# alibaba/TePDist

Hardware: AMD Instinct MI355X
Metric: tokens/sec (higher is better)
Workload: dtype bf16; 1 GPU; model=gpt2-345m, global_batch=64, seq_len=1024, parallelism=auto-planned-graph:dp1tp1pp1mesh[]micro1

## Files before the change

tepdist_amd/ops/csrc/bindings.cpp:

```cpp

#include <pybind11/pybind11.h>

#include <hip/hip_runtime.h>

#include "common.h"
#include "gemm_plan.h"
#include "kernels.h"

namespace py = pybind11;
using namespace tepdist;

namespace {

hipStream_t S(uintptr_t s) { return reinterpret_cast<hipStream_t>(s); }

void check_launch() { HIP_CHECK(hipGetLastError()); }

}

PYBIND11_MODULE(_tepdist_hip, m) {
  m.doc() = "TePDist-AMD gfx950 kernel library";

  m.def("gemm", [](uintptr_t A, uintptr_t B, uintptr_t C, uintptr_t Cpre,
                   uintptr_t bias, int M, int N, int K, int lda, int ldb,
                   int ldc, int64_t sa, int64_t sb, int64_t sc, int batch,
                   bool a_kc, bool b_kc, int epi, uintptr_t splitk_ws,
                   uintptr_t stream) {
    gemm_bf16(reinterpret_cast<void*>(A), reinterpret_cast<void*>(B),
              reinterpret_cast<void*>(C), reinterpret_cast<void*>(Cpre),
              reinterpret_cast<void*>(bias), M, N, K, lda, ldb, ldc, sa, sb,
              sc, batch, a_kc, b_kc, epi, reinterpret_cast<float*>(splitk_ws),
              S(stream));
    check_launch();
  });

  m.def("gemm_plan", [](int M, int N, int K, int lda, int ldb, bool a_kc,
                        bool b_kc, int epi, int batch) {
    const GemmPlan p = gemm_plan(M, N, K, lda, ldb, a_kc, b_kc, epi, batch);
    return py::make_tuple(p.kernel, p.split_k, p.k_chunk,
                          p.why_not ? p.why_not : "");
  }, py::arg("M"), py::arg("N"), py::arg("K"), py::arg("lda"),
     py::arg("ldb"), py::arg("a_kc") = true, py::arg("b_kc") = true,
     py::arg("epi") = 0, py::arg("batch") = 1);

  m.def("transpose", [](uintptr_t in, uintptr_t out, int R, int C,
                        int64_t si, int64_t so, int batch,
                        uintptr_t stream) {
    transpose_bf16(reinterpret_cast<void*>(in), reinterpret_cast<void*>(out),
                   R, C, si, so, batch, S(stream));
    check_launch();
  });

  m.def("layernorm_fwd", [](uintptr_t x, uintptr_t g, uintptr_t b, uintptr_t y,
                            uintptr_t mean, uintptr_t rstd, int rows, int cols,
                            float eps, uintptr_t stream, uintptr_t res,
                            uintptr_t sum_out) {
    layernorm_fwd_bf16(reinterpret_cast<void*>(x), reinterpret_cast<void*>(g),
                       reinterpret_cast<void*>(b), reinterpret_cast<void*>(y),
                       reinterpret_cast<float*>(mean),
                       reinterpret_cast<float*>(rstd), rows, cols, eps,
                       S(stream), reinterpret_cast<void*>(res),
                       reinterpret_cast<void*>(sum_out));
    check_launch();
  }, pybind11::arg("x"), pybind11::arg("g"), pybind11::arg("b"),
     pybind11::arg("y"), pybind11::arg("mean"), pybind11::arg("rstd"),
     pybind11::arg("rows"), pybind11::arg("cols"), pybind11::arg("eps"),
     pybind11::arg("stream"), pybind11::arg("res") = 0,
     pybind11::arg("sum_out") = 0);

  m.def("layernorm_bwd", [](uintptr_t dy, uintptr_t x, uintptr_t g,
                            uintptr_t mean, uintptr_t rstd, uintptr_t dx,
                            uintptr_t dg_part, uintptr_t db_part,
                            uintptr_t dgamma, uintptr_t dbeta, int rows,
                            int cols, int part_rows, uintptr_t stream,
                            uintptr_t dsum) {
    layernorm_bwd_bf16(reinterpret_cast<void*>(dy), reinterpret_cast<void*>(x),
                       reinterpret_cast<void*>(g),
                       reinterpret_cast<float*>(mean),
                       reinterpret_cast<float*>(rstd),
                       reinterpret_cast<void*>(dx),
                       reinterpret_cast<float*>(dg_part),
                       reinterpret_cast<float*>(db_part), rows, cols,
                       part_rows, S(stream), reinterpret_cast<void*>(dsum));
    check_launch();
    layernorm_bwd_reduce(reinterpret_cast<float*>(dg_part),
                         reinterpret_cast<float*>(db_part),
                         reinterpret_cast<void*>(dgamma),
// ... 299 lines not shown
```

tepdist_amd/ops/csrc/gemm.hip:

```cpp

#include <algorithm>
#include <stdexcept>
#include <string>

#include "common.h"
#include "gemm_tile.h"
#include "kernels.h"

namespace tepdist {

namespace {

constexpr int BM = plan::T128, BN = plan::T128, BK = plan::BK;
constexpr int SLOT = BM * BK;
constexpr int NTHREADS = 256;

DEV_INLINE int lds_off(int row, int col_e) { return loff<BK>(row, col_e); }


DEV_INLINE void stage_kc_load(const bf16_t* __restrict__ src, int F, int K,
                              int ld, int f0, int k0, bool aligned,
                              bf16x8 regs[4]) {
#pragma unroll
  for (int u = 0; u < 4; ++u) {
// ... 188 lines not shown
#pragma unroll
      for (int i = 0; i < 4; ++i) {
        af[i] = frag(sa, wm + i * 16, lane, kk);
        bfr[i] = frag(sb, wn + i * 16, lane, kk);
      }
#pragma unroll
      for (int mi = 0; mi < 4; ++mi)
#pragma unroll
        for (int ni = 0; ni < 4; ++ni)
          acc[mi][ni] = __builtin_amdgcn_mfma_f32_16x16x32_bf16(
              af[mi], bfr[ni], acc[mi][ni], 0, 0, 0);
    }

    if (t + 1 < nk) write_tiles(cur ^ 1, kbeg + (t + 1) * BK);
    __syncthreads();
  }

  float bv[4];
  if (EPI == EPI_BIAS || EPI == EPI_BIAS_GELU) {
#pragma unroll
    for (int ni = 0; ni < 4; ++ni) {
      const int n = n0 + wn + ni * 16 + (lane & 15);
      bv[ni] = (n < N) ? bf2f(bias[n]) : 0.0f;
    }
  }
#pragma unroll
  for (int mi = 0; mi < 4; ++mi) {
#pragma unroll
    for (int ni = 0; ni < 4; ++ni) {
      const int n = n0 + wn + ni * 16 + (lane & 15);
      if (n >= N) continue;
#pragma unroll
      for (int e = 0; e < 4; ++e) {
        const int m = m0 + wm + mi * 16 + (lane >> 4) * 4 + e;
        if (m >= M) continue;
        float v = acc[mi][ni][e];
        if (EPI == EPI_BIAS || EPI == EPI_BIAS_GELU) v += bv[ni];
        const int64_t off = (int64_t)m * ldc + n;
        if (F32OUT) {
          Cf[off] = v;
          continue;
        }
        if (EPI >= 2) {
          const bf16_t pre = f2bf(v);
          Cpre[off] = pre;
          v = gelu_f(bf2f(pre));
        }
        C[off] = f2bf(v);
      }
    }
  }
}

__global__ void splitk_reduce_kernel(const float* __restrict__ parts,
                                     bf16_t* __restrict__ out, int nparts,
                                     int64_t mn) {
  const int64_t stride = (int64_t)gridDim.x * blockDim.x * 4;
  for (int64_t i = ((int64_t)blockIdx.x * blockDim.x + threadIdx.x) * 4;
       i < mn; i += stride) {
    if (i + 4 <= mn) {
      f32x4 sv = *reinterpret_cast<const f32x4*>(parts + i);
      for (int p = 1; p < nparts; ++p) {
        const f32x4 v = *reinterpret_cast<const f32x4*>(parts + p * mn + i);
#pragma unroll
        for (int e = 0; e < 4; ++e) sv[e] += v[e];
      }
      bf16x4 o;
#pragma unroll
      for (int e = 0; e < 4; ++e) o[e] = f2bf(sv[e]);
      *reinterpret_cast<bf16x4*>(out + i) = o;
    } else {
      for (int64_t j = i; j < mn; ++j) {
        float acc = 0.f;
        for (int p = 0; p < nparts; ++p) acc += parts[p * mn + j];
        out[j] = f2bf(acc);
      }
    }
  }
}

void splitk_reduce(const float* parts, bf16_t* out, int nparts, int64_t mn,
                   hipStream_t stream) {
  const int blocks = (int)std::min<int64_t>(
      (mn / 4 + NTHREADS - 1) / NTHREADS, 2048);
  hipLaunchKernelGGL(splitk_reduce_kernel, dim3(std::max(blocks, 1)),
                     dim3(NTHREADS), 0, stream, parts, out, nparts, mn);
}

}

void gemm_bf16(const void* A, const void* B, void* C, void* c_pre,
               const void* bias, int M, int N, int K, int lda, int ldb,
               int ldc, int64_t stride_a, int64_t stride_b, int64_t stride_c,
               int batch, bool a_kc, bool b_kc, int epi, float* splitk_ws,
               hipStream_t stream) {
  const GemmPlan p = gemm_plan(M, N, K, lda, ldb, a_kc, b_kc, epi, batch);
  if (p.kernel == 0)
    throw std::runtime_error(std::string("gemm_bf16: ") + p.why_not);

  const bool split = p.split_k > 1;
  const int64_t mn = (int64_t)M * N;
  if (split && splitk_ws == nullptr)
    throw std::runtime_error("gemm_bf16: split-K plan needs a workspace of " +
                             std::to_string(p.split_k * mn) + " floats");
  if (split && ldc != N)
    throw std::runtime_error("gemm_bf16: split-K plan needs ldc == N");
  void* out = C;
  if (split) {
    out = splitk_ws;
    stride_c = mn;
  }

  if (p.kernel == plan::T256) {
    gemm256_bf16(A, B, out, c_pre, bias, M, N, K, lda, ldb, ldc, stride_a,
                 stride_b, stride_c, batch, !a_kc, epi, p.split_k,
                 p.k_chunk, stream);
  } else {
    const int nbx = (N + BN - 1) / BN, nby = (M + BM - 1) / BM;
    const dim3 grid(nbx * nby, 1, split ? p.split_k : batch), block(NTHREADS);
    const bf16_t* a = static_cast<const bf16_t*>(A);
    const bf16_t* b = static_cast<const bf16_t*>(B);
    bf16_t* cp = static_cast<bf16_t*>(c_pre);
    const bf16_t* bi = static_cast<const bf16_t*>(bias);
#define GEMM_LAUNCH(AKC, BKC, E, F32)                                       \
    hipLaunchKernelGGL((gemm_kernel<AKC, BKC, E, F32>), grid, block, 0,     \
                       stream, a, b, out, cp, bi, M, N, K, lda, ldb, ldc,   \
                       stride_a, stride_b, stride_c, p.k_chunk)
#define GEMM_EPI(AKC, BKC)                                                  \
    if (split) { GEMM_LAUNCH(AKC, BKC, 0, true); }                          \
    else switch (epi) {                  \
      case EPI_NONE: GEMM_LAUNCH(AKC, BKC, EPI_NONE, false); break;         \
      case EPI_BIAS: GEMM_LAUNCH(AKC, BKC, EPI_BIAS, false); break;         \
      case EPI_BIAS_GELU: GEMM_LAUNCH(AKC, BKC, EPI_BIAS_GELU, false); break; \
      case EPI_GELU: GEMM_LAUNCH(AKC, BKC, EPI_GELU, false); break;         \
    }
    if (a_kc && b_kc) { GEMM_EPI(true, true); }
    else if (a_kc && !b_kc) { GEMM_EPI(true, false); }
    else if (!a_kc && b_kc) { GEMM_EPI(false, true); }
    else { GEMM_EPI(false, false); }
#undef GEMM_EPI
#undef GEMM_LAUNCH
  }
  if (split) {
    HIP_CHECK(hipGetLastError());
    splitk_reduce(splitk_ws, static_cast<bf16_t*>(C), p.split_k, mn, stream);
  }
}

}
```

tepdist_amd/ops/csrc/gemm256.hip:

```cpp

#include <stdexcept>

#include "common.h"
#include "gemm_tile.h"
#include "kernels.h"

namespace tepdist {

namespace {

constexpr int BM = plan::T256, BN = plan::T256, BK = plan::BK;
constexpr int NTH = 512;
constexpr int QROWS = 64;
constexpr int SLOT_E = QROWS * BK;

DEV_INLINE int qoff(int row, int col_e) { return loff<BK>(row, col_e); }

DEV_INLINE void stage_q(const bf16_t* __restrict__ src, int64_t ld, int f0,
                        int k0, bf16_t* dst) {
  const int wave = threadIdx.x >> 6;
  const int row = threadIdx.x >> 3;
  const int c = (threadIdx.x & 7) * 8;
  const int ksrc = k0 + (c ^ (SWZ8(row) << 3));
  const bf16_t* g = src + (int64_t)(f0 + row) * ld + ksrc;
// ... 4 lines not shown
DEV_INLINE int qoff_f32(int row, int col_e) {
  return row * BK + (col_e ^ (SWZ8(row) << 2));
}

DEV_INLINE bf16x8 fragq(const bf16_t* slot, int row, int col_e) {
  return *reinterpret_cast<const bf16x8*>(slot + qoff(row, col_e));
}

typedef unsigned int u32x2 __attribute__((ext_vector_type(2)));
typedef __attribute__((address_space(3))) const bf16_t* lds_cptr_t;

template <int OFF>
DEV_INLINE bf16x4 tr_read_asm(uint32_t addr) {
  u32x2 v;
  asm volatile("ds_read_b64_tr_b16 %0, %1 offset:%2"
               : "=v"(v)
               : "v"(addr), "n"(OFF)
               : "memory");
  return __builtin_bit_cast(bf16x4, v);
}

template <int KK>
DEV_INLINE bf16x8 tr_frag_asm(const bf16_t* slot, int df, int lane) {
  const int i = lane & 15, g = lane >> 4;
  const uint32_t addr = (uint32_t)(uintptr_t)(lds_cptr_t)(
      slot + qoff(4 * g + (i >> 2), 16 * df + 4 * (i & 3)));
  const bf16x4 lo = tr_read_asm<KK * 32 * BK * 2>(addr);
  const bf16x4 hi = tr_read_asm<(KK * 32 + 16) * BK * 2>(addr);
  bf16x8 f;
#pragma unroll
  for (int e = 0; e < 4; ++e) {
    f[e] = lo[e];
    f[e + 4] = hi[e];
  }
  return f;
}

template <bool KO, int KK>
DEV_INLINE bf16x8 frag_fk(const bf16_t* slot, int df, int lane) {
  if (KO) return tr_frag_asm<KK>(slot, df, lane);
  return fragq(slot, df * 16 + (lane & 15), 8 * (lane >> 4) + 32 * KK);
}

#define RAW_BAR() __builtin_amdgcn_s_barrier()
#define VMCNT6() asm volatile("s_waitcnt vmcnt(6)" ::: "memory")
#define LGKM_WAIT_KO()                                      \
  do {                                                      \
    if (KO) {                                               \
      asm volatile("s_waitcnt lgkmcnt(0)" ::: "memory");    \
      __builtin_amdgcn_sched_barrier(0);                    \
    }                                                       \
  } while (0)

template <int EPI, bool F32OUT = false, bool KO = false>
__launch_bounds__(NTH, 1) __global__
void gemm256_kernel(const bf16_t* __restrict__ A,
                    const bf16_t* __restrict__ B, void* __restrict__ Cv,
                    bf16_t* __restrict__ Cpre,
                    const bf16_t* __restrict__ bias, int M, int N, int K,
                    int lda, int ldb, int ldc, int64_t strideA,
                    int64_t strideB, int64_t strideC, int k_chunk) {
  bf16_t* C = static_cast<bf16_t*>(Cv);
  float* Cf = static_cast<float*>(Cv);
  int kbeg = 0, kend = K;
  if (F32OUT) {
    kbeg = blockIdx.z * k_chunk;
    kend = min(K, kbeg + k_chunk);
    Cf += blockIdx.z * strideC;
    if (kend <= kbeg) kbeg = kend = 0;
  } else {
    A += blockIdx.z * strideA;
    B += blockIdx.z * strideB;
    C += blockIdx.z * strideC;
    if (EPI >= 2) Cpre += blockIdx.z * strideC;
  }

  const int nbx = N / BN;
  const int swz = xcd_remap(blockIdx.x, gridDim.x);
  const int m0 = (swz / nbx) * BM, n0 = (swz % nbx) * BN;

  __shared__ bf16_t smem[16 * SLOT_E];
  bf16_t* const aslot = smem;
  bf16_t* const bslot = smem + 8 * SLOT_E;

  const int lane = threadIdx.x & 63;
  const int wm = (threadIdx.x >> 8) & 1;
  const int wn = (threadIdx.x >> 6) & 3;

  f32x4 acc[8][4] = {};

  const int nk = (kend - kbeg) / BK;

  auto stage_1 = [&](const bf16_t* __restrict__ src, int ld, int f0, int t,
                     bf16_t* dst) {
    if (KO) stage_q(src, ld, kbeg + t * BK, f0, dst);
    else    stage_q(src, ld, f0, kbeg + t * BK, dst);
  };
  auto stage_a = [&](int t, int q2) {
    stage_1(A, lda, m0 + 64 * q2, t, aslot + ((4 * t + q2) & 7) * SLOT_E);
    stage_1(A, lda, m0 + 64 * (q2 + 1), t,
            aslot + ((4 * t + q2 + 1) & 7) * SLOT_E);
  };
  auto stage_b = [&](int t, int q2) {
    stage_1(B, ldb, n0 + 64 * q2, t, bslot + ((4 * t + q2) & 7) * SLOT_E);
    stage_1(B, ldb, n0 + 64 * (q2 + 1), t,
            bslot + ((4 * t + q2 + 1) & 7) * SLOT_E);
  };

  if (nk > 0) {
    stage_a(0, 0);
    stage_a(0, 2);
    stage_b(0, 0);
    stage_b(0, 2);
    if (nk > 1) {
      stage_a(1, 0);
      stage_a(1, 2);
      stage_b(1, 0);
    }
    VMCNT6();
  }
  RAW_BAR();

  bf16x8 af[8][2];
  for (int t = 0; t < nk; ++t) {
    if (t + 1 == nk && nk > 1) {
      asm volatile("s_waitcnt vmcnt(0)" ::: "memory");
      RAW_BAR();
    }
    {
      const bf16_t* as0 = aslot + ((4 * t + 2 * wm) & 7) * SLOT_E;
      const bf16_t* as1 = aslot + ((4 * t + 2 * wm + 1) & 7) * SLOT_E;
#pragma unroll
      for (int mi = 0; mi < 8; ++mi) {
        const bf16_t* s = (mi < 4) ? as0 : as1;
        af[mi][0] = frag_fk<KO, 0>(s, mi & 3, lane);
        af[mi][1] = frag_fk<KO, 1>(s, mi & 3, lane);
      }
      bf16x8 bf0[2];
      {
        const bf16_t* bs = bslot + ((4 * t + 0) & 7) * SLOT_E;
        bf0[0] = frag_fk<KO, 0>(bs, wn, lane);
        bf0[1] = frag_fk<KO, 1>(bs, wn, lane);
      }
      if (t + 1 < nk) stage_b(t + 1, 2);
      RAW_BAR();
      LGKM_WAIT_KO();
      __builtin_amdgcn_s_setprio(1);
#pragma unroll
      for (int mi = 0; mi < 8; ++mi)
#pragma unroll
        for (int kk = 0; kk < 2; ++kk)
          acc[mi][0] = __builtin_amdgcn_mfma_f32_16x16x32_bf16(
              af[mi][kk], bf0[kk], acc[mi][0], 0, 0, 0);
      __builtin_amdgcn_s_setprio(0);
      RAW_BAR();
    }
#pragma unroll
    for (int p = 1; p < 4; ++p) {
      bf16x8 bfp[2];
      {
        const bf16_t* bs = bslot + ((4 * t + p) & 7) * SLOT_E;
        bfp[0] = frag_fk<KO, 0>(bs, wn, lane);
        bfp[1] = frag_fk<KO, 1>(bs, wn, lane);
      }
      if (p == 1 && t + 2 < nk) stage_a(t + 2, 0);
      if (p == 2 && t + 2 < nk) stage_a(t + 2, 2);
      if (p == 3 && t + 2 < nk) stage_b(t + 2, 0);
      RAW_BAR();
      LGKM_WAIT_KO();
      __builtin_amdgcn_s_setprio(1);
#pragma unroll
      for (int mi = 0; mi < 8; ++mi)
#pragma unroll
        for (int kk = 0; kk < 2; ++kk)
          acc[mi][p] = __builtin_amdgcn_mfma_f32_16x16x32_bf16(
              af[mi][kk], bfp[kk], acc[mi][p], 0, 0, 0);
      __builtin_amdgcn_s_setprio(0);
      if (p == 3) VMCNT6();
      RAW_BAR();
    }
  }

  float bv[4];
  if (EPI == EPI_BIAS || EPI == EPI_BIAS_GELU) {
#pragma unroll
    for (int p = 0; p < 4; ++p)
      bv[p] = bf2f(bias[n0 + 64 * p + wn * 16 + (lane & 15)]);
  }
  if (!F32OUT) {
    asm volatile("s_waitcnt lgkmcnt(0)" ::: "memory");
    __builtin_amdgcn_s_barrier();
    bf16_t* img = smem;
#pragma unroll
    for (int p = 0; p < 4; ++p) {
      const int cl = wn * 16 + (lane & 15);
#pragma unroll
      for (int mi = 0; mi < 8; ++mi)
#pragma unroll
        for (int e = 0; e < 4; ++e) {
          const int row = wm * 128 + mi * 16 + (lane >> 4) * 4 + e;
          float v = acc[mi][p][e];
          if (EPI == EPI_BIAS || EPI == EPI_BIAS_GELU) v += bv[p];
          img[qoff(row, cl)] = f2bf(v);
        }
      asm volatile("s_waitcnt lgkmcnt(0)" ::: "memory");
      __builtin_amdgcn_s_barrier();
      const int sr = threadIdx.x >> 3;
      const int c8 = (threadIdx.x & 7) * 8;
#pragma unroll
      for (int rr = 0; rr < BM; rr += 64) {
        const int row = rr + sr;
        const int64_t off = (int64_t)(m0 + row) * ldc + n0 + 64 * p + c8;
        bf16x8 v8 = *reinterpret_cast<const bf16x8*>(img + qoff(row, c8));
        if (EPI == EPI_DGELU) {
          const bf16x8 pv = *reinterpret_cast<const bf16x8*>(Cpre + off);
#pragma unroll
          for (int e = 0; e < 8; ++e)
            v8[e] = f2bf(bf2f(v8[e]) * gelu_grad_f(bf2f(pv[e])));
        } else if (EPI >= 2) {
          *reinterpret_cast<bf16x8*>(Cpre + off) = v8;
#pragma unroll
          for (int e = 0; e < 8; ++e) v8[e] = f2bf(gelu_f(bf2f(v8[e])));
        }
        *reinterpret_cast<bf16x8*>(C + off) = v8;
      }
      asm volatile("s_waitcnt lgkmcnt(0)" ::: "memory");
      __builtin_amdgcn_s_barrier();
    }
    return;
  }
  asm volatile("s_waitcnt lgkmcnt(0)" ::: "memory");
  __builtin_amdgcn_s_barrier();
  {
    float* imgf = reinterpret_cast<float*>(smem);
#pragma unroll
    for (int p = 0; p < 4; ++p) {
      const int cl = wn * 16 + (lane & 15);
#pragma unroll
      for (int mi = 0; mi < 8; ++mi)
#pragma unroll
        for (int e = 0; e < 4; ++e) {
          const int row = wm * 128 + mi * 16 + (lane >> 4) * 4 + e;
          imgf[qoff_f32(row, cl)] = acc[mi][p][e];
        }
      asm volatile("s_waitcnt lgkmcnt(0)" ::: "memory");
      __builtin_amdgcn_s_barrier();
      const int sr = threadIdx.x >> 4;
      const int c4 = (threadIdx.x & 15) * 4;
#pragma unroll
      for (int rr = 0; rr < BM; rr += 32) {
        const int row = rr + sr;
        const int64_t off = (int64_t)(m0 + row) * ldc + n0 + 64 * p + c4;
        *reinterpret_cast<f32x4*>(Cf + off) =
            *reinterpret_cast<const f32x4*>(imgf + qoff_f32(row, c4));
      }
      asm volatile("s_waitcnt lgkmcnt(0)" ::: "memory");
      __builtin_amdgcn_s_barrier();
    }
  }
}

}

void gemm256_bf16(const void* A, const void* B, void* C, void* c_pre,
                  const void* bias, int M, int N, int K, int lda, int ldb,
                  int ldc, int64_t stride_a, int64_t stride_b,
                  int64_t stride_c, int batch, bool k_outer, int epi,
                  int split_k, int k_chunk, hipStream_t stream) {
  const bool split = split_k > 1;
  const dim3 grid((N / BN) * (M / BM), 1, split ? split_k : batch), block(NTH);
  const bf16_t* a = static_cast<const bf16_t*>(A);
  const bf16_t* b = static_cast<const bf16_t*>(B);
  bf16_t* cp = static_cast<bf16_t*>(c_pre);
  const bf16_t* bi = static_cast<const bf16_t*>(bias);
#define G256(E, F32, KO)                                                    \
  hipLaunchKernelGGL((gemm256_kernel<E, F32, KO>), grid, block, 0, stream, \
                     a, b, C, cp, bi, M, N, K, lda, ldb, ldc, stride_a,    \
                     stride_b, stride_c, k_chunk)
  if (k_outer) {
    if (epi != EPI_NONE)
      throw std::runtime_error(
          "gemm256_bf16: k-outer operands have only the plain epilogue");
    if (split) { G256(EPI_NONE, true, true); }
    else { G256(EPI_NONE, false, true); }
  } else if (split) { G256(EPI_NONE, true, false); }
  else switch (epi) {
    case EPI_NONE: G256(EPI_NONE, false, false); break;
    case EPI_BIAS: G256(EPI_BIAS, false, false); break;
    case EPI_BIAS_GELU: G256(EPI_BIAS_GELU, false, false); break;
    case EPI_GELU: G256(EPI_GELU, false, false); break;
    case EPI_DGELU: G256(EPI_DGELU, false, false); break;
  }
#undef G256
}

}
```

tepdist_amd/ops/csrc/gemm_plan.h:

```cpp
#pragma once

#include <algorithm>
#include <cstdint>

namespace tepdist {

struct GemmPlan {
  int kernel;
  int split_k;
  int k_chunk;
  const char* why_not;
};

enum {
  EPI_NONE = 0,
  EPI_BIAS = 1,
  EPI_BIAS_GELU = 2,
  EPI_GELU = 3,
  EPI_DGELU = 4
};

namespace plan {
constexpr int T256 = 256;
constexpr int T128 = 128;
// ... 11 lines not shown
    int s = std::max(2, (512 + b - 1) / b);
    for (int cand = s; cand < std::min(17, max_by_k + 1); ++cand)
      if ((b * cand) % 256 == 0) {
        s = cand;
        break;
      }
    s = std::max(2, std::min({s, 16, max_by_k}));
    const int64_t floor_chunk = cdiv(K / s, BK) * BK;
    *split_k = static_cast<int>(std::max<int64_t>(2, cdiv(K, floor_chunk)));
    *k_chunk = static_cast<int>(cdiv(cdiv(K, *split_k), BK) * BK);
  }
}

inline bool chunks_fit_256(int K, int split_k, int k_chunk) {
  if (K < 2 * BK) return false;
  if (split_k == 1) return true;
  return k_chunk >= 2 * BK && K % k_chunk != BK &&
         cdiv(K, k_chunk) == split_k;
}
}

inline GemmPlan gemm_plan(int M, int N, int K, int lda, int ldb, bool a_kc,
                          bool b_kc, int epi, int batch) {
  using namespace plan;
  if (epi < EPI_NONE || epi > EPI_DGELU)
    return {0, 1, 0, "epi must be 0..4"};

  const bool tiled = M % T256 == 0 && N % T256 == 0 && K % BK == 0;
  const bool canon = a_kc && b_kc && tiled;
  const bool aligned = (lda & 7) == 0 && (ldb & 7) == 0;
  int split_k, k_chunk;

  if (!a_kc && !b_kc && tiled && aligned && epi == EPI_NONE) {
    split_for(int64_t(M / T256) * (N / T256), K, epi, batch, &split_k,
              &k_chunk);
    if (chunks_fit_256(K, split_k, k_chunk))
      return {T256, split_k, k_chunk, nullptr};
  }

  const int64_t blocks = canon ? int64_t(M / T256) * (N / T256)
                               : cdiv(M, T128) * cdiv(N, T128);
  split_for(blocks, K, epi, batch, &split_k, &k_chunk);

  if (canon && aligned && chunks_fit_256(K, split_k, k_chunk))
    return {T256, split_k, k_chunk, nullptr};
  if (epi == EPI_DGELU)
    return {0, 1, 0,
            "epi 4 (dgelu) runs only on the 256 kernel: k-contiguous "
            "operands, M and N multiples of 256, K a multiple of 64 and "
            ">= 128, 16-byte-aligned rows"};
  return {T128, split_k, k_chunk, nullptr};
}

}
```

tepdist_amd/ops/csrc/kernels.h:

```cpp
#pragma once

#include <hip/hip_runtime.h>
#include <hip/hip_bf16.h>
#include <cstdint>

namespace tepdist {

using bf16 = __hip_bfloat16;

void gemm_bf16(const void* A, const void* B, void* C, void* c_pre,
               const void* bias, int M, int N, int K, int lda, int ldb,
               int ldc, int64_t stride_a, int64_t stride_b, int64_t stride_c,
               int batch, bool a_kc, bool b_kc, int epi, float* splitk_ws,
               hipStream_t stream);
void gemm256_bf16(const void* A, const void* B, void* C, void* c_pre,
                  const void* bias, int M, int N, int K, int lda, int ldb,
                  int ldc, int64_t stride_a, int64_t stride_b,
                  int64_t stride_c, int batch, bool k_outer, int epi,
                  int split_k, int k_chunk, hipStream_t stream);

void transpose_bf16(const void* in, void* out, int R, int C,
                    int64_t stride_in, int64_t stride_out, int batch,
                    hipStream_t stream);
void cast_ws_f32_bf16(const float* ws, void* db_out, int cols,
                      hipStream_t stream);
void transpose_dy_bf16(const void* dy, const void* pre, void* dy_t,
                       void* dy_nat, float* bias_ws, int R, int C,
                       hipStream_t stream);

void layernorm_fwd_bf16(const void* x, const void* gamma, const void* beta,
                        void* y, float* mean, float* rstd, int rows, int cols,
                        float eps, hipStream_t stream,
                        const void* res = nullptr, void* sum_out = nullptr);
void layernorm_bwd_bf16(const void* dy, const void* x, const void* gamma,
                        const float* mean, const float* rstd, void* dx,
                        float* dgamma_part, float* dbeta_part, int rows,
                        int cols, int part_rows, hipStream_t stream,
                        const void* dsum = nullptr);
void layernorm_bwd_reduce(const float* dgamma_part, const float* dbeta_part,
                          void* dgamma, void* dbeta, int part_rows, int cols,
                          hipStream_t stream);

void softmax_fwd_bf16(const void* x, void* p, int64_t rows, int cols, int sq,
                      float scale, bool causal, hipStream_t stream);
void softmax_bwd_bf16(const void* dp, const void* p, void* ds, int64_t rows,
                      int cols, float scale, hipStream_t stream);

void attention_fwd_bf16(const void* q, const void* k, const void* v, void* o,
                        float* lse, int B, int H, int S, int D, float scale,
                        bool causal, int64_t q_bs, int64_t q_hs, int64_t q_rs,
                        int64_t o_bs, int64_t o_hs, int64_t o_rs,
                        hipStream_t stream);
void attention_bwd_bf16(const void* q, const void* k, const void* v,
                        const void* o, const void* dout, const float* lse,
                        float* delta, void* dq, void* dk, void* dv,
                        int B, int H, int S, int D, float scale, bool causal,
                        int64_t q_bs, int64_t q_hs, int64_t q_rs,
                        int64_t o_bs, int64_t o_hs, int64_t o_rs,
                        hipStream_t stream);

void decode_attention_bf16(const void* q, const void* k_new,
                           const void* v_new, void* k_cache, void* v_cache,
                           const int64_t* pos, int pos_stride, void* out,
                           float* ws, int B, int H, int Hkv, int S_max,
                           int D, float scale, int splits, bool rope,
                           float rope_theta, int64_t q_bs,
                           int64_t q_hs, int64_t n_bs, int64_t n_hs,
                           int64_t c_bs, int64_t c_hs, int64_t c_rs,
                           hipStream_t stream);

int64_t moe_route_ws_ints(int T, int E);
void moe_route(const void* gates, bool gates_fp32, int* topi, int* slot,
// ... 67 lines not shown
```

tepdist_amd/ops/hip.py:

```python

from __future__ import annotations

import math
import os
from typing import Optional, Tuple

import torch

try:
    from tepdist_amd.ops import _tepdist_hip as ext
except ImportError as e:
    raise ImportError(
        "tepdist_amd HIP extension not built. Run "
        "`python tepdist_amd/ops/build_ext.py` (hipcc cross-compiles on a "
        "GPU-less box). No eager fallback is provided on GPU.") from e

BF16 = torch.bfloat16


def _stream() -> int:
    return torch.cuda.current_stream().cuda_stream


def _p(t: Optional[torch.Tensor]) -> int:
    return 0 if t is None else t.data_ptr()


def _layout2d(t: torch.Tensor, kc_expected_inner: bool):
    assert t.dim() == 2
    if t.stride(1) == 1:
        return True, t.stride(0)
    if t.stride(0) == 1:
        return False, t.stride(1)
    raise ValueError(f"operand must be contiguous in one dim, strides={t.stride()}")



_GEMM_BACKEND = os.environ.get("TEPDIST_GEMM_BACKEND", "auto")
_gemm_choice = {}


def _pick_backend(key, hip_fn, blt_fn):
    if _GEMM_BACKEND == "hip":
        return hip_fn
    if _GEMM_BACKEND == "blaslt":
        return blt_fn
    got = _gemm_choice.get(key)
    if got is not None:
        return hip_fn if got == "hip" else blt_fn
    if torch.cuda.is_current_stream_capturing():
        return hip_fn
    import time as _time

    def _t(fn):
        fn()
        fn()
        torch.cuda.synchronize()
        best = float("inf")
        for _ in range(3):
            t0 = _time.perf_counter()
            fn()
            fn()
            torch.cuda.synchronize()
            best = min(best, _time.perf_counter() - t0)
        return best

    th, tb = _t(hip_fn), _t(blt_fn)
    _gemm_choice[key] = "hip" if th <= tb else "blaslt"
    return hip_fn if th <= tb else blt_fn


def _gemm_raw(a: torch.Tensor, b_stored: torch.Tensor, a_kc: bool, b_kc: bool,
              M: int, N: int, K: int, lda: int, ldb: int,
              sa: int, sb: int, batch: int, bias=None, epi: int = 0,
              out=None, out_pre=None, device=None):
    dev = device if device is not None else a.device
    c = out if out is not None else torch.empty(
        (batch, M, N) if batch > 1 else (M, N), dtype=BF16, device=dev)
    cp = out_pre
    if epi >= 2 and cp is None:
        cp = torch.empty_like(c)

    split_k = ext.gemm_plan(M, N, K, lda, ldb, a_kc, b_kc, epi, batch)[1]
    ws = torch.empty(split_k * M * N, dtype=torch.float32, device=dev) \
        if split_k > 1 else None
    ext.gemm(a.data_ptr(), b_stored.data_ptr(), c.data_ptr(), _p(cp), _p(bias),
             M, N, K, lda, ldb, N, sa, sb, M * N, batch, a_kc, b_kc, epi,
             _p(ws), _stream())
    return c, cp


def linear_fwd(x: torch.Tensor, w: torch.Tensor, bias: Optional[torch.Tensor],
               act: str = "none") -> Tuple[torch.Tensor, Optional[torch.Tensor]]:
    assert x.dtype == BF16 and w.dtype == BF16, "hip backend is bf16-only"
    x = x.contiguous()
    M, K = x.shape
    N = w.shape[0]
    if act == "none":
        epi = 1 if bias is not None else 0
    elif act == "gelu":
        epi = 2 if bias is not None else 3
    else:
        raise ValueError(act)

    def _hip():
        return _gemm_raw(x, w, True, True, M, N, K, K, w.stride(0), 0, 0, 1,
                         bias=bias, epi=epi)

    def _blt():
        pre = torch.nn.functional.linear(x, w, bias)
        if act != "gelu":
            return pre, None
        y = torch.empty_like(pre)
        ext.gelu_fwd(pre.data_ptr(), y.data_ptr(), pre.numel(), _stream())
        return y, pre

    fn = _pick_backend(("lin_f", M, N, K, epi), _hip, _blt)
    return fn()


def _bias_sum(t: torch.Tensor) -> torch.Tensor:
    rows, cols = t.shape
    db = torch.empty(cols, dtype=BF16, device=t.device)
    ws = torch.zeros(cols, dtype=torch.float32, device=t.device)
    ext.bias_sum(t.data_ptr(), db.data_ptr(), ws.data_ptr(), rows, cols,
                 _stream())
    return db


def gelu_fwd(x: torch.Tensor) -> torch.Tensor:
    x = x.contiguous()
    y = torch.empty_like(x)
    ext.gelu_fwd(x.data_ptr(), y.data_ptr(), x.numel(), _stream())
    return y


def gelu_bwd(dy: torch.Tensor, x: torch.Tensor) -> torch.Tensor:
    dy, x = dy.contiguous(), x.contiguous()
    dx = torch.empty_like(dy)
    ext.gelu_bwd(dy.data_ptr(), x.data_ptr(), dx.data_ptr(), dy.numel(),
                 _stream())
# ... 22 lines not shown
def _blt_mlp_dgelu(dy: torch.Tensor, w2: torch.Tensor, pre: torch.Tensor):
    M, N = dy.shape
    K = w2.shape[1]
    dh = torch.empty(M, K, dtype=BF16, device=dy.device)
    db1 = torch.empty(K, dtype=BF16, device=dy.device)
    _blt.blt_fused(1, M, N, K, w2.data_ptr(), dy.data_ptr(), dh.data_ptr(),
                   db1.data_ptr(), pre.data_ptr(), _stream())
    return dh, db1


_blt_ok = True


def _blt_usable() -> bool:
    return _blt is not None and _blt_ok and _MLP_FUSED != "0"


def mlp_fwd(x, w1, b1, w2, b2):
    global _blt_ok
    x = x.contiguous()
    res = {}

    def _fused():
        h, pre = _blt_mlp_gelu(x, w1, b1)
        res["h"], res["pre"] = h, pre
        return linear_fwd(h, w2, b2, "none")[0]

    def _composed():
        h, pre = linear_fwd(x, w1, b1, "gelu")
        res["h"], res["pre"] = h, pre
        return linear_fwd(h, w2, b2, "none")[0]

    if not _blt_usable():
        y = _composed()
    elif _MLP_FUSED == "1":
        y = _fused()
    else:
        try:
            y = _pick_backend(("mlp_f", x.shape[0], w1.shape[0],
                               x.shape[1]), _fused, _composed)()
        except RuntimeError:
            _blt_ok = False
            y = _composed()
    return y, (res["h"], res["pre"])


def mlp_bwd(dy, x, w1, w2, h, pre):
    global _blt_ok
    dy = dy.contiguous()
    out = {}

    def _fused():
        dh, db1 = _blt_mlp_dgelu(dy, w2, pre)
        dw2 = matmul(dy.t(), h)
        db2 = _bias_sum(dy)
        dx, dw1, _ = linear_bwd(dh, x, w1, False, "none", None)
        out["r"] = (dx, dw1, db1, dw2, db2)

    def _composed():
        dh_post, dw2, db2 = linear_bwd(dy, h, w2, True, "none", None)
        dx, dw1, db1 = linear_bwd(dh_post, x, w1, True, "gelu", pre)
        out["r"] = (dx, dw1, db1, dw2, db2)

    def _hand_dgelu():
        M, N2 = dy.shape
        K2 = w2.shape[1]
        w2T = transpose2d(w2)
        dh, _ = _gemm_raw(dy, w2T, True, True, M, K2, N2, N2, N2, 0, 0, 1,
                          epi=4, out_pre=pre)
        db1 = _bias_sum(dh)
        dw2 = matmul(dy.t(), h)
        db2 = _bias_sum(dy)
        dx, dw1, _ = linear_bwd(dh, x, w1, False, "none", None)
        out["r"] = (dx, dw1, db1, dw2, db2)

    def _base():
        M, N2 = dy.shape
        K2 = w2.shape[1]
        if (ext.gemm_plan(M, K2, N2, N2, N2, True, True, 4, 1)[0] == 256
                and pre.is_contiguous()):
            _pick_backend(("mlp_bh", dy.shape[0], dy.shape[1],
                           w2.shape[1]), _hand_dgelu, _composed)()
        else:
            _composed()

    if not _blt_usable():
        _base()
    elif _MLP_FUSED == "1":
        _fused()
    else:
        try:
            _pick_backend(("mlp_b", dy.shape[0], dy.shape[1],
                           w2.shape[1]), _fused, _base)()
        except RuntimeError:
            _blt_ok = False
            _base()
    return out["r"]


def transpose2d(t: torch.Tensor) -> torch.Tensor:
    R, C = t.shape[-2], t.shape[-1]
    batch = t.numel() // (R * C)
    t = t.contiguous()
    out = torch.empty((*t.shape[:-2], C, R), dtype=t.dtype, device=t.device)
    ext.transpose(t.data_ptr(), out.data_ptr(), R, C, R * C, R * C, batch,
                  _stream())
    return out


def linear_bwd(dy: torch.Tensor, x: torch.Tensor, w: torch.Tensor,
               has_bias: bool, act: str, pre_act: Optional[torch.Tensor]):
    dy = dy.contiguous()
    M, N = dy.shape
    K = w.shape[1]

    if x.stride(-1) == 1 and \
            ext.gemm_plan(N, K, M, N, x.stride(0), False, False, 0, 1)[0] == 256:
        if act == "gelu":
            dyl = torch.empty_like(dy)
            ext.gelu_bwd(dy.data_ptr(), pre_act.data_ptr(), dyl.data_ptr(),
                         dy.numel(), _stream())
        else:
            dyl = dy

        def _dx_hip():
            wT = transpose2d(w)
            return _gemm_raw(dyl, wT, True, True, M, K, N, N, N, 0, 0, 1)[0]

        def _dw_hip():
            return _gemm_raw(dyl, x, False, False, N, K, M, N, x.stride(0),
                             0, 0, 1)[0]

        dx = _pick_backend(("lin_bx", M, N, K), _dx_hip,
                           lambda: torch.matmul(dyl, w))()
        dw = _pick_backend(("lin_bw", M, N, K), _dw_hip,
                           lambda: torch.matmul(dyl.t(), x))()
        return dx, dw, _bias_sum(dyl) if has_bias else None

    def _hip():
        dyl = dy
        wT = transpose2d(w)
        dyT = torch.empty(N, M, dtype=BF16, device=dy.device)
        if act == "gelu":
            dy_eff = torch.empty_like(dyl)
            ext.transpose_dy(dyl.data_ptr(), pre_act.data_ptr(),
                             dyT.data_ptr(), dy_eff.data_ptr(), 0, M, N,
                             _stream())
            dyl = dy_eff
        else:
            ext.transpose_dy(dyl.data_ptr(), 0, dyT.data_ptr(), 0, 0, M, N,
                             _stream())
        xT = transpose2d(x)
        dx, _ = _gemm_raw(dyl, wT, True, True, M, K, N, N, N, 0, 0, 1)
        dw, _ = _gemm_raw(dyT, xT, True, True, N, K, M, M, M, 0, 0, 1)
        return dx, dw, dyl

    def _blt():
        if act == "gelu":
            dyl = torch.empty_like(dy)
            ext.gelu_bwd(dy.data_ptr(), pre_act.data_ptr(), dyl.data_ptr(),
                         dy.numel(), _stream())
        else:
            dyl = dy
        dx = torch.matmul(dyl, w)
        dw = torch.matmul(dyl.t(), x)
        return dx, dw, dyl

    fn = _pick_backend(("lin_b", M, N, K, act), _hip, _blt)
    dx, dw, dy_eff = fn()
    db = None
    if has_bias:
        db = _bias_sum(dy_eff)
    return dx, dw, db


def matmul(a: torch.Tensor, b: torch.Tensor) -> torch.Tensor:
    key = ("mm", tuple(a.shape), tuple(b.shape),
           a.stride(-1) == 1, b.stride(-1) == 1)
    return _pick_backend(key, lambda: _matmul_hip(a, b),
                         lambda: torch.matmul(a, b))()


def _matmul_hip(a: torch.Tensor, b: torch.Tensor) -> torch.Tensor:
    assert a.dtype == BF16 and b.dtype == BF16
    squeeze = a.dim() == 2 and b.dim() == 2
    lead_shape = (a if a.dim() >= b.dim() else b).shape[:-2]
    if a.dim() == 2:
        a = a.unsqueeze(0)
    if b.dim() == 2:
        b = b.unsqueeze(0)
# ... 650 lines not shown
```

Baseline: 320,500 tokens/s.

## Fuse bias-gradient column sums into the weight-gradient GEMM via MFMA with ones

Adds a column-sum path to the 256-tile GEMM for k-outer operands. While computing dW = dy^T x, one column of tiles multiplies the A fragments by a vector of ones through MFMA to produce partial bias gradients. These partials are reduced in a small kernel, or inside the split-K reduce launch, so the separate bias_sum pass over dy is no longer needed. The weight-gradient wrapper is shared by the MLP and linear backward paths and picks the backend by autotune. In exchange it adds extra MFMA work, a larger workspace, and a new template variant that may raise register pressure.

```diff
diff --git a/tepdist_amd/ops/csrc/bindings.cpp b/tepdist_amd/ops/csrc/bindings.cpp
--- a/tepdist_amd/ops/csrc/bindings.cpp
+++ b/tepdist_amd/ops/csrc/bindings.cpp
@@ -2,6 +2,9 @@
 #include <pybind11/pybind11.h>
 
 #include <hip/hip_runtime.h>
+
+#include <stdexcept>
+#include <string>
 
 #include "common.h"
 #include "gemm_plan.h"
@@ -25,14 +28,31 @@
                    uintptr_t bias, int M, int N, int K, int lda, int ldb,
                    int ldc, int64_t sa, int64_t sb, int64_t sc, int batch,
                    bool a_kc, bool b_kc, int epi, uintptr_t splitk_ws,
-                   uintptr_t stream) {
+                   uintptr_t stream, uintptr_t colsum_out) {
     gemm_bf16(reinterpret_cast<void*>(A), reinterpret_cast<void*>(B),
               reinterpret_cast<void*>(C), reinterpret_cast<void*>(Cpre),
               reinterpret_cast<void*>(bias), M, N, K, lda, ldb, ldc, sa, sb,
               sc, batch, a_kc, b_kc, epi, reinterpret_cast<float*>(splitk_ws),
-              S(stream));
-    check_launch();
-  });
+              reinterpret_cast<void*>(colsum_out), S(stream));
+    check_launch();
+  }, py::arg("A"), py::arg("B"), py::arg("C"), py::arg("Cpre"),
+     py::arg("bias"), py::arg("M"), py::arg("N"), py::arg("K"),
+     py::arg("lda"), py::arg("ldb"), py::arg("ldc"), py::arg("sa"),
+     py::arg("sb"), py::arg("sc"), py::arg("batch"), py::arg("a_kc"),
+     py::arg("b_kc"), py::arg("epi"), py::arg("splitk_ws"),
+     py::arg("stream"), py::arg("colsum_out") = 0);
+
+  m.def("gemm_ws_floats", [](int M, int N, int K, int lda, int ldb,
+                             bool a_kc, bool b_kc, int epi, int batch,
+                             bool colsum) {
+    const GemmPlan p = gemm_plan(M, N, K, lda, ldb, a_kc, b_kc, epi, batch);
+    if (colsum)
+      if (const char* why = colsum_why_not(p, a_kc, b_kc, batch))
+        throw std::runtime_error(std::string("gemm_ws_floats: ") + why);
+    return gemm_ws_floats(p, M, N, colsum);
+  }, py::arg("M"), py::arg("N"), py::arg("K"), py::arg("lda"),
+     py::arg("ldb"), py::arg("a_kc") = true, py::arg("b_kc") = true,
+     py::arg("epi") = 0, py::arg("batch") = 1, py::arg("colsum") = false);
 
   m.def("gemm_plan", [](int M, int N, int K, int lda, int ldb, bool a_kc,
                         bool b_kc, int epi, int batch) {
diff --git a/tepdist_amd/ops/csrc/gemm.hip b/tepdist_amd/ops/csrc/gemm.hip
--- a/tepdist_amd/ops/csrc/gemm.hip
+++ b/tepdist_amd/ops/csrc/gemm.hip
@@ -264,11 +264,50 @@
   }
 }
 
+constexpr int CS_COLS = 32, CS_GROUPS = NTHREADS / CS_COLS;
+
+DEV_INLINE void colsum_reduce(const float* __restrict__ parts,
+                              bf16_t* __restrict__ out, int nparts, int m,
+                              int blk, float* sh) {
+  const int c = threadIdx.x % CS_COLS, g = threadIdx.x / CS_COLS;
+  const int i = blk * CS_COLS + c;
+  float acc = 0.f;
+  if (i < m) {
+#pragma unroll 4
+    for (int p = g; p < nparts; p += CS_GROUPS)
+      acc += parts[(int64_t)p * m + i];
+  }
+  sh[g * CS_COLS + c] = acc;
+  __syncthreads();
+  if (g == 0 && i < m) {
+    float s = sh[c];
+#pragma unroll
+    for (int q = 1; q < CS_GROUPS; ++q) s += sh[q * CS_COLS + c];
+    out[i] = f2bf(s);
+  }
+}
+
+__global__ void colsum_reduce_kernel(const float* __restrict__ parts,
+                                     bf16_t* __restrict__ out, int nparts,
+                                     int m) {
+  __shared__ float sh[NTHREADS];
+  colsum_reduce(parts, out, nparts, m, blockIdx.x, sh);
+}
+
 __global__ void splitk_reduce_kernel(const float* __restrict__ parts,
                                      bf16_t* __restrict__ out, int nparts,
-                                     int64_t mn) {
-  const int64_t stride = (int64_t)gridDim.x * blockDim.x * 4;
-  for (int64_t i = ((int64_t)blockIdx.x * blockDim.x + threadIdx.x) * 4;
+                                     int64_t mn, int cs_blocks,
+                                     const float* __restrict__ cs_parts,
+                                     bf16_t* __restrict__ cs_out,
+                                     int cs_nparts, int cs_m) {
+  __shared__ float sh[NTHREADS];
+  if ((int)blockIdx.x < cs_blocks) {
+    colsum_reduce(cs_parts, cs_out, cs_nparts, cs_m, blockIdx.x, sh);
+    return;
+  }
+  const int blk = blockIdx.x - cs_blocks;
+  const int64_t stride = (int64_t)(gridDim.x - cs_blocks) * blockDim.x * 4;
+  for (int64_t i = ((int64_t)blk * blockDim.x + threadIdx.x) * 4;
        i < mn; i += stride) {
     if (i + 4 <= mn) {
       f32x4 sv = *reinterpret_cast<const f32x4*>(parts + i);
@@ -292,11 +331,14 @@
 }
 
 void splitk_reduce(const float* parts, bf16_t* out, int nparts, int64_t mn,
-                   hipStream_t stream) {
-  const int blocks = (int)std::min<int64_t>(
-      (mn / 4 + NTHREADS - 1) / NTHREADS, 2048);
-  hipLaunchKernelGGL(splitk_reduce_kernel, dim3(std::max(blocks, 1)),
-                     dim3(NTHREADS), 0, stream, parts, out, nparts, mn);
+                   const float* cs_parts, bf16_t* cs_out, int cs_nparts,
+                   int cs_m, hipStream_t stream) {
+  const int blocks = std::max(1, (int)std::min<int64_t>(
+      (mn / 4 + NTHREADS - 1) / NTHREADS, 2048));
+  const int cs_blocks = cs_out ? (cs_m + CS_COLS - 1) / CS_COLS : 0;
+  hipLaunchKernelGGL(splitk_reduce_kernel, dim3(cs_blocks + blocks),
+                     dim3(NTHREADS), 0, stream, parts, out, nparts, mn,
+                     cs_blocks, cs_parts, cs_out, cs_nparts, cs_m);
 }
 
 }
@@ -305,16 +347,26 @@
                const void* bias, int M, int N, int K, int lda, int ldb,
                int ldc, int64_t stride_a, int64_t stride_b, int64_t stride_c,
                int batch, bool a_kc, bool b_kc, int epi, float* splitk_ws,
-               hipStream_t stream) {
+               void* colsum_out, hipStream_t stream) {
   const GemmPlan p = gemm_plan(M, N, K, lda, ldb, a_kc, b_kc, epi, batch);
   if (p.kernel == 0)
     throw std::runtime_error(std::string("gemm_bf16: ") + p.why_not);
+  const bool colsum = colsum_out != nullptr;
+  if (colsum) {
+    if (const char* why = colsum_why_not(p, a_kc, b_kc, batch))
+      throw std::runtime_error(std::string("gemm_bf16: ") + why);
+    if (splitk_ws == nullptr)
+      throw std::runtime_error(
+          "gemm_bf16: colsum_out needs a workspace of " +
+          std::to_string(gemm_ws_floats(p, M, N, true)) + " floats");
+  }
 
   const bool split = p.split_k > 1;
   const int64_t mn = (int64_t)M * N;
   if (split && splitk_ws == nullptr)
     throw std::runtime_error("gemm_bf16: split-K plan needs a workspace of " +
-                             std::to_string(p.split_k * mn) + " floats");
+                             std::to_string(gemm_ws_floats(p, M, N, false)) +
+                             " floats");
   if (split && ldc != N)
     throw std::runtime_error("gemm_bf16: split-K plan needs ldc == N");
   void* out = C;
@@ -322,11 +374,14 @@
     out = splitk_ws;
     stride_c = mn;
   }
+  float* cs_parts =
+      colsum ? splitk_ws + gemm_ws_floats(p, M, N, false) : nullptr;
+  const int cs_nparts = p.split_k * (N / plan::T256);
 
   if (p.kernel == plan::T256) {
     gemm256_bf16(A, B, out, c_pre, bias, M, N, K, lda, ldb, ldc, stride_a,
                  stride_b, stride_c, batch, !a_kc, epi, p.split_k,
-                 p.k_chunk, stream);
+                 p.k_chunk, cs_parts, stream);
   } else {
     const int nbx = (N + BN - 1) / BN, nby = (M + BM - 1) / BM;
     const dim3 grid(nbx * nby, 1, split ? p.split_k : batch), block(NTHREADS);
@@ -355,8 +410,16 @@
   }
   if (split) {
     HIP_CHECK(hipGetLastError());
-    splitk_reduce(splitk_ws, static_cast<bf16_t*>(C), p.split_k, mn, stream);
-  }
-}
-
-}
+    splitk_reduce(splitk_ws, static_cast<bf16_t*>(C), p.split_k, mn,
+                  cs_parts, static_cast<bf16_t*>(colsum_out), cs_nparts, M,
+                  stream);
+  } else if (colsum) {
+    HIP_CHECK(hipGetLastError());
+    hipLaunchKernelGGL(colsum_reduce_kernel,
+                       dim3((M + CS_COLS - 1) / CS_COLS), dim3(NTHREADS), 0,
+                       stream, cs_parts, static_cast<bf16_t*>(colsum_out),
+                       cs_nparts, M);
+  }
+}
+
+}
diff --git a/tepdist_amd/ops/csrc/gemm256.hip b/tepdist_amd/ops/csrc/gemm256.hip
--- a/tepdist_amd/ops/csrc/gemm256.hip
+++ b/tepdist_amd/ops/csrc/gemm256.hip
@@ -80,14 +80,16 @@
     }                                                       \
   } while (0)
 
-template <int EPI, bool F32OUT = false, bool KO = false>
+template <int EPI, bool F32OUT = false, bool KO = false, bool CS = false>
 __launch_bounds__(NTH, 1) __global__
 void gemm256_kernel(const bf16_t* __restrict__ A,
                     const bf16_t* __restrict__ B, void* __restrict__ Cv,
                     bf16_t* __restrict__ Cpre,
                     const bf16_t* __restrict__ bias, int M, int N, int K,
                     int lda, int ldb, int ldc, int64_t strideA,
-                    int64_t strideB, int64_t strideC, int k_chunk) {
+                    int64_t strideB, int64_t strideC, int k_chunk,
+                    float* __restrict__ colsum) {
+  static_assert(!CS || (KO && EPI == EPI_NONE), "CS: k-outer, plain epilogue");
   bf16_t* C = static_cast<bf16_t*>(Cv);
   float* Cf = static_cast<float*>(Cv);
   int kbeg = 0, kend = K;
@@ -149,6 +151,15 @@
   }
   RAW_BAR();
 
+  const int cs_wn = CS ? __builtin_amdgcn_readfirstlane(wn) : 0;
+  int cs_next = swz % nbx;
+  f32x4 cs[2] = {};
+  bf16x8 ones;
+  if (CS) {
+#pragma unroll
+    for (int e = 0; e < 8; ++e) ones[e] = f2bf(1.0f);
+  }
+
   bf16x8 af[8][2];
   for (int t = 0; t < nk; ++t) {
     if (t + 1 == nk && nk > 1) {
@@ -180,6 +191,19 @@
         for (int kk = 0; kk < 2; ++kk)
           acc[mi][0] = __builtin_amdgcn_mfma_f32_16x16x32_bf16(
               af[mi][kk], bf0[kk], acc[mi][0], 0, 0, 0);
+      if (CS && t == cs_next) {
+        cs_next += nbx;
+#pragma unroll
+        for (int w = 0; w < 4; ++w)
+          if (w == cs_wn) {
+#pragma unroll
+            for (int kk = 0; kk < 2; ++kk)
+#pragma unroll
+              for (int h = 0; h < 2; ++h)
+                cs[h] = __builtin_amdgcn_mfma_f32_16x16x32_bf16(
+                    af[2 * w + h][kk], ones, cs[h], 0, 0, 0);
+          }
+      }
       __builtin_amdgcn_s_setprio(0);
       RAW_BAR();
     }
@@ -206,6 +230,16 @@
       __builtin_amdgcn_s_setprio(0);
       if (p == 3) VMCNT6();
       RAW_BAR();
+    }
+  }
+
+  if (CS) {
+    float* part = colsum +
+        ((int64_t)(F32OUT ? blockIdx.z : 0) * nbx + swz % nbx) * M + m0 +
+        wm * 128 + wn * 32 + 4 * (lane >> 4);
+    if ((lane & 15) == 0) {
+      *reinterpret_cast<f32x4*>(part) = cs[0];
+      *reinterpret_cast<f32x4*>(part + 16) = cs[1];
     }
   }
 
@@ -294,30 +328,40 @@
                   const void* bias, int M, int N, int K, int lda, int ldb,
                   int ldc, int64_t stride_a, int64_t stride_b,
                   int64_t stride_c, int batch, bool k_outer, int epi,
-                  int split_k, int k_chunk, hipStream_t stream) {
+                  int split_k, int k_chunk, float* colsum_parts,
+                  hipStream_t stream) {
   const bool split = split_k > 1;
   const dim3 grid((N / BN) * (M / BM), 1, split ? split_k : batch), block(NTH);
   const bf16_t* a = static_cast<const bf16_t*>(A);
   const bf16_t* b = static_cast<const bf16_t*>(B);
   bf16_t* cp = static_cast<bf16_t*>(c_pre);
   const bf16_t* bi = static_cast<const bf16_t*>(bias);
-#define G256(E, F32, KO)                                                    \
-  hipLaunchKernelGGL((gemm256_kernel<E, F32, KO>), grid, block, 0, stream, \
-                     a, b, C, cp, bi, M, N, K, lda, ldb, ldc, stride_a,    \
-                     stride_b, stride_c, k_chunk)
+#define G256(E, F32, KO, CS)                                               \
+  hipLaunchKernelGGL((gemm256_kernel<E, F32, KO, CS>), grid, block, 0,     \
+                     stream, a, b, C, cp, bi, M, N, K, lda, ldb, ldc,      \
+                     stride_a, stride_b, stride_c, k_chunk, colsum_parts)
   if (k_outer) {
     if (epi != EPI_NONE)
       throw std::runtime_error(
           "gemm256_bf16: k-outer operands have only the plain epilogue");
-    if (split) { G256(EPI_NONE, true, true); }
-    else { G256(EPI_NONE, false, true); }
-  } else if (split) { G256(EPI_NONE, true, false); }
+    if (colsum_parts && batch != 1)
+      throw std::runtime_error("gemm256_bf16: column sums need batch 1");
+    if (colsum_parts) {
+      if (split) { G256(EPI_NONE, true, true, true); }
+      else { G256(EPI_NONE, false, true, true); }
+    }
+    else if (split) { G256(EPI_NONE, true, true, false); }
+    else { G256(EPI_NONE, false, true, false); }
+  } else if (colsum_parts) {
+    throw std::runtime_error(
+        "gemm256_bf16: column sums need two k-outer operands");
+  } else if (split) { G256(EPI_NONE, true, false, false); }
   else switch (epi) {
-    case EPI_NONE: G256(EPI_NONE, false, false); break;
-    case EPI_BIAS: G256(EPI_BIAS, false, false); break;
-    case EPI_BIAS_GELU: G256(EPI_BIAS_GELU, false, false); break;
-    case EPI_GELU: G256(EPI_GELU, false, false); break;
-    case EPI_DGELU: G256(EPI_DGELU, false, false); break;
+    case EPI_NONE: G256(EPI_NONE, false, false, false); break;
+    case EPI_BIAS: G256(EPI_BIAS, false, false, false); break;
+    case EPI_BIAS_GELU: G256(EPI_BIAS_GELU, false, false, false); break;
+    case EPI_GELU: G256(EPI_GELU, false, false, false); break;
+    case EPI_DGELU: G256(EPI_DGELU, false, false, false); break;
   }
 #undef G256
 }
diff --git a/tepdist_amd/ops/csrc/gemm_plan.h b/tepdist_amd/ops/csrc/gemm_plan.h
--- a/tepdist_amd/ops/csrc/gemm_plan.h
+++ b/tepdist_amd/ops/csrc/gemm_plan.h
@@ -87,4 +87,19 @@
   return {T128, split_k, k_chunk, nullptr};
 }
 
+inline const char* colsum_why_not(const GemmPlan& p, bool a_kc, bool b_kc,
+                                  int batch) {
+  if (p.kernel != plan::T256 || a_kc || b_kc || batch != 1)
+    return "colsum_out needs the 256 kernel on two k-outer operands (A "
+           "stored [K][M], B stored [K][N], M and N multiples of 256, K a "
+           "multiple of 64 and >= 128, 16-byte-aligned rows, epi 0, batch 1)";
+  return nullptr;
 }
+
+inline int64_t gemm_ws_floats(const GemmPlan& p, int M, int N, bool colsum) {
+  int64_t n = p.split_k > 1 ? int64_t(p.split_k) * M * N : 0;
+  if (colsum) n += int64_t(p.split_k) * (N / plan::T256) * M;
+  return n;
+}
+
+}
diff --git a/tepdist_amd/ops/csrc/kernels.h b/tepdist_amd/ops/csrc/kernels.h
--- a/tepdist_amd/ops/csrc/kernels.h
+++ b/tepdist_amd/ops/csrc/kernels.h
@@ -12,12 +12,13 @@
                const void* bias, int M, int N, int K, int lda, int ldb,
                int ldc, int64_t stride_a, int64_t stride_b, int64_t stride_c,
                int batch, bool a_kc, bool b_kc, int epi, float* splitk_ws,
-               hipStream_t stream);
+               void* colsum_out, hipStream_t stream);
 void gemm256_bf16(const void* A, const void* B, void* C, void* c_pre,
                   const void* bias, int M, int N, int K, int lda, int ldb,
                   int ldc, int64_t stride_a, int64_t stride_b,
                   int64_t stride_c, int batch, bool k_outer, int epi,
-                  int split_k, int k_chunk, hipStream_t stream);
+                  int split_k, int k_chunk, float* colsum_parts,
+                  hipStream_t stream);
 
 void transpose_bf16(const void* in, void* out, int R, int C,
                     int64_t stride_in, int64_t stride_out, int batch,
diff --git a/tepdist_amd/ops/hip.py b/tepdist_amd/ops/hip.py
--- a/tepdist_amd/ops/hip.py
+++ b/tepdist_amd/ops/hip.py
@@ -73,7 +73,7 @@
 def _gemm_raw(a: torch.Tensor, b_stored: torch.Tensor, a_kc: bool, b_kc: bool,
               M: int, N: int, K: int, lda: int, ldb: int,
               sa: int, sb: int, batch: int, bias=None, epi: int = 0,
-              out=None, out_pre=None, device=None):
+              out=None, out_pre=None, device=None, colsum_out=None):
     dev = device if device is not None else a.device
     c = out if out is not None else torch.empty(
         (batch, M, N) if batch > 1 else (M, N), dtype=BF16, device=dev)
@@ -81,12 +81,13 @@
     if epi >= 2 and cp is None:
         cp = torch.empty_like(c)
 
-    split_k = ext.gemm_plan(M, N, K, lda, ldb, a_kc, b_kc, epi, batch)[1]
-    ws = torch.empty(split_k * M * N, dtype=torch.float32, device=dev) \
-        if split_k > 1 else None
+    ws_floats = ext.gemm_ws_floats(M, N, K, lda, ldb, a_kc, b_kc, epi, batch,
+                                   colsum_out is not None)
+    ws = torch.empty(ws_floats, dtype=torch.float32, device=dev) \
+        if ws_floats else None
     ext.gemm(a.data_ptr(), b_stored.data_ptr(), c.data_ptr(), _p(cp), _p(bias),
              M, N, K, lda, ldb, N, sa, sb, M * N, batch, a_kc, b_kc, epi,
-             _p(ws), _stream())
+             _p(ws), _stream(), _p(colsum_out))
     return c, cp
 
 
@@ -215,8 +216,7 @@
 
     def _fused():
         dh, db1 = _blt_mlp_dgelu(dy, w2, pre)
-        dw2 = matmul(dy.t(), h)
-        db2 = _bias_sum(dy)
+        dw2, db2 = wgrad(dy, h, True)
         dx, dw1, _ = linear_bwd(dh, x, w1, False, "none", None)
         out["r"] = (dx, dw1, db1, dw2, db2)
 
@@ -232,8 +232,7 @@
         dh, _ = _gemm_raw(dy, w2T, True, True, M, K2, N2, N2, N2, 0, 0, 1,
                           epi=4, out_pre=pre)
         db1 = _bias_sum(dh)
-        dw2 = matmul(dy.t(), h)
-        db2 = _bias_sum(dy)
+        dw2, db2 = wgrad(dy, h, True)
         dx, dw1, _ = linear_bwd(dh, x, w1, False, "none", None)
         out["r"] = (dx, dw1, db1, dw2, db2)
 
@@ -271,14 +270,41 @@
     return out
 
 
+def _wgrad_in_place(dyl: torch.Tensor, x: torch.Tensor) -> bool:
+    (M, N), K = dyl.shape, x.shape[1]
+    return dyl.stride(-1) == 1 and x.stride(-1) == 1 and ext.gemm_plan(
+        N, K, M, dyl.stride(0), x.stride(0), False, False, 0, 1)[0] == 256
+
+
+def wgrad(dyl: torch.Tensor, x: torch.Tensor, has_bias: bool):
+    M, N = dyl.shape
+    K = x.shape[1]
+    def _db():
+        return _bias_sum(dyl.contiguous()) if has_bias else None
+
+    if not _wgrad_in_place(dyl, x):
+        return matmul(dyl.t(), x), _db()
+
+    def _hand():
+        db = torch.empty(N, dtype=BF16, device=dyl.device) \
+            if has_bias else None
+        dw = _gemm_raw(dyl, x, False, False, N, K, M, dyl.stride(0),
+                       x.stride(0), 0, 0, 1, colsum_out=db)[0]
+        return dw, db
+
+    def _lib():
+        return torch.matmul(dyl.t(), x), _db()
+
+    return _pick_backend(("lin_bw", M, N, K, has_bias), _hand, _lib)()
+
+
 def linear_bwd(dy: torch.Tensor, x: torch.Tensor, w: torch.Tensor,
                has_bias: bool, act: str, pre_act: Optional[torch.Tensor]):
     dy = dy.contiguous()
     M, N = dy.shape
     K = w.shape[1]
 
-    if x.stride(-1) == 1 and \
-            ext.gemm_plan(N, K, M, N, x.stride(0), False, False, 0, 1)[0] == 256:
+    if _wgrad_in_place(dy, x):
         if act == "gelu":
             dyl = torch.empty_like(dy)
             ext.gelu_bwd(dy.data_ptr(), pre_act.data_ptr(), dyl.data_ptr(),
@@ -290,15 +316,10 @@
             wT = transpose2d(w)
             return _gemm_raw(dyl, wT, True, True, M, K, N, N, N, 0, 0, 1)[0]
 
-        def _dw_hip():
-            return _gemm_raw(dyl, x, False, False, N, K, M, N, x.stride(0),
-                             0, 0, 1)[0]
-
         dx = _pick_backend(("lin_bx", M, N, K), _dx_hip,
                            lambda: torch.matmul(dyl, w))()
-        dw = _pick_backend(("lin_bw", M, N, K), _dw_hip,
-                           lambda: torch.matmul(dyl.t(), x))()
-        return dx, dw, _bias_sum(dyl) if has_bias else None
+        dw, db = wgrad(dyl, x, has_bias)
+        return dx, dw, db
 
     def _hip():
         dyl = dy
```

After: 329,900 tokens/s (median of 6 runs). 2.9% higher.
